# harryjfowen/PointsToWood

Measured on AMD Instinct MI355X. Metric: classified points/sec, higher is better.
Workload: dtype f16x3

## Files before the change

pointstowood_amd/csrc/p2w_hgemm.h:

```cpp
#pragma once
#include "p2w_common.h"
#include <type_traits>

typedef float f32x16 __attribute__((ext_vector_type(16)));
typedef _Float16 h8 __attribute__((ext_vector_type(8)));
typedef __bf16 bf8 __attribute__((ext_vector_type(8)));
typedef __fp16 hpair __attribute__((ext_vector_type(2)));
typedef _Float16 hpairn __attribute__((ext_vector_type(2)));
typedef __bf16 bpair __attribute__((ext_vector_type(2)));
typedef float fpair __attribute__((ext_vector_type(2)));
typedef __attribute__((address_space(3))) void* lds_vp;
typedef const __attribute__((address_space(1))) void* glb_vp;

constexpr int H_BK = 32;
constexpr int SA_EPI_COLS = 1024;

template <int PREC> struct HCfg {
    static constexpr int planes = PREC == 0 ? 2 : 1;
    static constexpr int kslab = PREC == 0 ? 32 : 64;
    static constexpr int kalign = PREC == 0 ? 32 : 64;
};

template <int PREC>
__device__ __forceinline__ f32x16 h_mfma(h8 a, h8 b, f32x16 c) {
// ... 56 lines not shown
        w.y = pack_pair<PREC>(v[2], v[3]);
        *reinterpret_cast<uint2*>(base + row * (size_t)ldh + col) = w;
    }
}

__device__ __forceinline__ bool tile_coords_at(int L, int nMt, int nNt, int* mt, int* nt, int mode = 0) {
    const int xcd = L & 7, w = L >> 3;
    if (mode == 0) {
        *mt = xcd + 8 * (w / nNt);
        *nt = w % nNt;
        return *mt < nMt;
    }
    if (nNt >= 8) {
        const int cpx = (nNt + 7) >> 3;
        *mt = w / cpx;
        *nt = xcd + 8 * (w % cpx);
        return *mt < nMt && *nt < nNt;
    }
    const int r = 8 / nNt;
    *nt = xcd % nNt;
    *mt = xcd / nNt + r * w;
    return *mt < nMt;
}
__device__ __forceinline__ bool tile_coords(int nMt, int nNt, int* mt, int* nt, int mode = 0) {
    return tile_coords_at(blockIdx.x, nMt, nNt, mt, nt, mode);
}
static inline int tile_grid(int nMt, int nNt, int mode = 0) {
    if (mode == 0) return 8 * ((nMt + 7) / 8) * nNt;
    if (nNt >= 8) return 8 * nMt * ((nNt + 7) / 8);
    const int r = 8 / nNt;
    return 8 * ((nMt + r - 1) / r);
}
static inline int p2w_cu_count() {
    int dev = 0, n = 256;
    if (hipGetDevice(&dev) == hipSuccess) hipDeviceGetAttribute(&n, hipDeviceAttributeMultiprocessorCount, dev);
    return n > 0 ? n : 256;
}

constexpr int RI_DEPTH = 2;
struct EpiArgs {
    const float *bias, *sc0, *sh0, *sc1, *sh1, *residual;
    int ldr, relu0, relu1, relu2, relu_final;
    const _Float16* res_h;
    unsigned* range;
    const int4* imeta;
};
__device__ __forceinline__ void range_commit(unsigned* __restrict__ dst, bool over, bool seen, int lane) {
    if (lane == 0) {
        unsigned* p = dst + (blockIdx.x & (P2W_RANGE_SLOTS - 1)) * 64;
        if (over) p[0] = 1u;
        if (seen) p[1] = 1u;
    }
}
__device__ __forceinline__ float nan_max(float a, float b) { return __builtin_elementwise_maximum(a, b); }
__device__ __forceinline__ void range_commit_max(unsigned* __restrict__ dst, float m, int lane) {
    range_commit(dst, __ballot(!(m <= P2W_RANGE_HI)) != 0ull, __ballot(m > P2W_RANGE_LO) != 0ull, lane);
}
template <int PREC>
__device__ __forceinline__ fpair h_load2(const _Float16* __restrict__ base, unsigned ldh, unsigned row, unsigned col) {
    if constexpr (PREC == 0) {
        const _Float16* p = base + (size_t)row * (2 * ldh) + 64 * (col >> 5) + (col & 31);
        const hpairn hi = *reinterpret_cast<const hpairn*>(p), lo = *reinterpret_cast<const hpairn*>(p + 32);
        return fpair{(float)hi[0] + (float)lo[0], (float)hi[1] + (float)lo[1]};
    } else if constexpr (PREC == 1) {
        const hpairn v = *reinterpret_cast<const hpairn*>(base + (size_t)row * ldh + col);
        return fpair{(float)v[0], (float)v[1]};
    } else {
        const bpair v = *reinterpret_cast<const bpair*>(base + (size_t)row * ldh + col);
        return fpair{(float)v[0], (float)v[1]};
    }
}
struct OutArgs { float* f32; int ldo; _Float16* h2; int ldh; int hcols; const float* dotw; float* part; int ldpart; };

__device__ __forceinline__ float row16_sum(float v) {
    asm volatile("s_nop 4\n\t"
                 "v_add_f32_dpp %0, %0, %0 quad_perm:[1,0,3,2] row_mask:0xf bank_mask:0xf bound_ctrl:1\n\ts_nop 1\n\t"
                 "v_add_f32_dpp %0, %0, %0 quad_perm:[2,3,0,1] row_mask:0xf bank_mask:0xf bound_ctrl:1\n\ts_nop 1\n\t"
                 "v_add_f32_dpp %0, %0, %0 row_half_mirror row_mask:0xf bank_mask:0xf bound_ctrl:1\n\ts_nop 1\n\t"
                 "v_add_f32_dpp %0, %0, %0 row_mirror row_mask:0xf bank_mask:0xf bound_ctrl:1\n\ts_nop 1"
                 : "+v"(v));
    return v;
}

__device__ __forceinline__ int w_stage_row16(int rho) {
    const int t = rho >> 4, c = rho & 15;
    return 32 * (t >> 1) + 2 * c + (t & 1);
}

template <int PREC, int RT16, int CT16, int EF, bool DOTK = false>
__device__ __forceinline__ void gemm_epilogue_16(const f32x4 (&acc)[RT16][CT16], const EpiArgs& ep, float wscale, int row0, int col0,
                                                 int lane, int M, int N, const OutArgs& o, bool seen_report = true) {
    static_assert(CT16 % 2 == 0, "column tiles come in interleaved pairs");
    constexpr bool GEN = EF < 0;
    constexpr int JQ = CT16 / 2, NSTEP = RT16 * 4;
    const bool R0 = GEN ? ep.relu0 != 0 : (EF & 1) != 0, S0 = GEN ? ep.sc0 != nullptr : (EF & 2) != 0;
    const bool R1 = GEN ? ep.relu1 != 0 : (EF & 4) != 0, S1 = GEN ? ep.sc1 != nullptr : (EF & 8) != 0;
    const bool R2 = GEN ? ep.relu2 != 0 : (EF & 16) != 0;
    const bool RES = !DOTK && (GEN ? (ep.residual != nullptr || ep.res_h != nullptr) : (EF & 32) != 0);
    const bool RF = GEN ? ep.relu_final != 0 : (EF & 64) != 0, OF = GEN ? o.f32 != nullptr : (EF & 128) != 0;
    const bool OH = GEN ? o.h2 != nullptr : (EF & 256) != 0;
    const bool RH = RES && (GEN ? ep.res_h != nullptr : (EF & 1024) != 0);
    constexpr bool RI_OK = !DOTK && RT16 <= 4;
    const bool RI = RI_OK && RES && (GEN ? ep.imeta != nullptr : (EF & 2048) != 0);
    const bool DOT = DOTK && (GEN ? o.dotw != nullptr : (EF & 512) != 0);
    const int c16 = lane & 15, kg = lane >> 4;
    const int cb = col0 + 2 * c16;
    fpair bias[JQ], s0[JQ], t0[JQ], s1[JQ], t1[JQ], dw[JQ];
#pragma unroll
    for (int jq = 0; jq < JQ; ++jq) {
        const int c = cb + 32 * jq;
        bias[jq] = fpair{0.f, 0.f}; s0[jq] = fpair{1.f, 1.f}; t0[jq] = fpair{0.f, 0.f}; s1[jq] = fpair{1.f, 1.f}; t1[jq] = fpair{0.f, 0.f};
        dw[jq] = fpair{0.f, 0.f};
        if constexpr (GEN) {
#pragma unroll
            for (int e = 0; e < 2; ++e)
                if (c + e < N) {
                    if (ep.bias) bias[jq][e] = ep.bias[c + e];
                    if (S0) { s0[jq][e] = ep.sc0[c + e]; t0[jq][e] = ep.sh0[c + e]; }
                    if (S1) { s1[jq][e] = ep.sc1[c + e]; t1[jq][e] = ep.sh1[c + e]; }
                    if (DOT) dw[jq][e] = o.dotw[c + e];
                }
        } else {
            if (DOT) dw[jq] = *reinterpret_cast<const fpair*>(o.dotw + c);
            if (ep.bias) bias[jq] = *reinterpret_cast<const fpair*>(ep.bias + c);
            if (S0) { s0[jq] = *reinterpret_cast<const fpair*>(ep.sc0 + c); t0[jq] = *reinterpret_cast<const fpair*>(ep.sh0 + c); }
            if (S1) { s1[jq] = *reinterpret_cast<const fpair*>(ep.sc1 + c); t1[jq] = *reinterpret_cast<const fpair*>(ep.sh1 + c); }
        }
    }
    auto row_of = [&](int st) { return row0 + 16 * (st >> 2) + 4 * kg + (st & 3); };
    auto value = [&](float a, float b, float s0v, float t0v, float s1v, float t1v, float res) {
        float v = fmaf(a, wscale, b);
        if (R0) v = fmaxf(v, 0.f);
        if (S0) v = fmaf(v, s0v, t0v);
        if (R1) v = fmaxf(v, 0.f);
        if (S1) v = fmaf(v, s1v, t1v);
        if (R2) v = fmaxf(v, 0.f);
        if (RES) v += res;
        if (RF) v = fmaxf(v, 0.f);
        return v;
    };
    fpair rcur[JQ], rnxt[JQ];
    constexpr int RI_D = RI_OK ? (RI_DEPTH < NSTEP ? RI_DEPTH : NSTEP) : 1;
    fpair z0r[RI_D][RI_OK ? JQ : 1], z1r[RI_D][RI_OK ? JQ : 1];
    float a0r[RI_D], a1r[RI_D];
    int4 m_nxt = make_int4(0, 0, 0, 0);
    auto load_zrows = [&](int slot, const int4& mt) {
        const float* p0 = ep.residual + ((unsigned)mt.x * (unsigned)ep.ldr + (unsigned)cb);
        const float* p1 = ep.residual + ((unsigned)mt.y * (unsigned)ep.ldr + (unsigned)cb);
#pragma unroll
        for (int jq = 0; jq < (RI_OK ? JQ : 1); ++jq) {
            z0r[slot][jq] = *reinterpret_cast<const fpair*>(p0 + 32 * jq);
            z1r[slot][jq] = *reinterpret_cast<const fpair*>(p1 + 32 * jq);
        }
        a0r[slot] = __int_as_float(mt.z); a1r[slot] = __int_as_float(mt.w);
    };
    auto load_res = [&](fpair (&dst)[JQ], int st) {
        if (RH) {
#pragma unroll
            for (int jq = 0; jq < JQ; ++jq) dst[jq] = h_load2<PREC>(ep.res_h, (unsigned)ep.ldr, (unsigned)row_of(st), (unsigned)(cb + 32 * jq));
        } else {
            const float* rp = ep.residual + ((unsigned)row_of(st) * (unsigned)ep.ldr + (unsigned)cb);
#pragma unroll
            for (int jq = 0; jq < JQ; ++jq) dst[jq] = *reinterpret_cast<const fpair*>(rp + 32 * jq);
        }
    };
#pragma unroll
    for (int jq = 0; jq < JQ; ++jq) { rcur[jq] = fpair{0.f, 0.f}; rnxt[jq] = fpair{0.f, 0.f}; }
    if constexpr (!GEN) {
        if constexpr (RI_OK) {
            if (RI) {
                int4 m0[RI_D];
#pragma unroll
                for (int d = 0; d < RI_D; ++d) m0[d] = ep.imeta[row_of(d)];
                if (RI_D < NSTEP) m_nxt = ep.imeta[row_of(RI_D)];
#pragma unroll
                for (int d = 0; d < RI_D; ++d) load_zrows(d, m0[d]);
            }
        }
        if (RES && !RI) load_res(rcur, 0);
    }
    float dot4[4] = {0.f, 0.f, 0.f, 0.f};
    unsigned long long r_over = 0ull, r_seen = 0ull;
    float m4 = 0.f;
#pragma unroll
    for (int st = 0; st < NSTEP; ++st) {
        const int it = st >> 2, reg = st & 3;
        const int row = row_of(st);
        if constexpr (!GEN) {
            if constexpr (RI_OK) {
                if (RI) {
#pragma unroll
                    for (int jq = 0; jq < JQ; ++jq)
                        rcur[jq] = fpair{fmaf(a1r[st % RI_D], z1r[st % RI_D][jq][0], a0r[st % RI_D] * z0r[st % RI_D][jq][0]),
                                         fmaf(a1r[st % RI_D], z1r[st % RI_D][jq][1], a0r[st % RI_D] * z0r[st % RI_D][jq][1])};
                    if (st + RI_D < NSTEP) {
                        load_zrows(st % RI_D, m_nxt);
                        if (st + RI_D + 1 < NSTEP) m_nxt = ep.imeta[row_of(st + RI_D + 1)];
                    }
                }
            }
            if (RES && !RI && st + 1 < NSTEP) load_res(rnxt, st + 1);
            __builtin_amdgcn_sched_barrier(0);
            float* fp = OF ? o.f32 + ((unsigned)row * (unsigned)o.ldo + (unsigned)cb) : nullptr;
            _Float16* hp = nullptr;
            if (OH) {
                if constexpr (PREC == 0) hp = o.h2 + ((unsigned)row * (unsigned)(2 * o.ldh) + (unsigned)(64 * (cb >> 5) + (cb & 31)));
                else hp = o.h2 + ((unsigned)row * (unsigned)o.ldh + (unsigned)cb);
            }
            float dsum = 0.f;
#pragma unroll
            for (int jq = 0; jq < JQ; ++jq) {
                const float va = value(acc[it][2 * jq][reg], bias[jq][0], s0[jq][0], t0[jq][0], s1[jq][0], t1[jq][0], rcur[jq][0]);
                const float vb = value(acc[it][2 * jq + 1][reg], bias[jq][1], s0[jq][1], t0[jq][1], s1[jq][1], t1[jq][1], rcur[jq][1]);
                m4 = nan_max(nan_max(m4, fabsf(va)), fabsf(vb));
                if (DOT) dsum = fmaf(vb, dw[jq][1], fmaf(va, dw[jq][0], dsum));
                if (OF) *reinterpret_cast<fpair*>(fp + 32 * jq) = fpair{va, vb};
                if (OH) {
                    if constexpr (PREC == 0) {
                        unsigned hw, lw;
                        split_pair(va, vb, hw, lw);
                        *reinterpret_cast<unsigned*>(hp + 64 * jq) = hw;
                        *reinterpret_cast<unsigned*>(hp + 64 * jq + 32) = lw;
                    } else {
                        *reinterpret_cast<unsigned*>(hp + 32 * jq) = pack_pair<PREC>(va, vb);
                    }
                }
            }
            if (reg == 3) {
                r_over |= __ballot(!(m4 <= P2W_RANGE_HI));
                r_seen |= __ballot(m4 > P2W_RANGE_LO);
                m4 = 0.f;
            }
            if (DOT) {
                dot4[reg] = row16_sum(dsum);
                if (reg == 3 && c16 == 0)
                    *reinterpret_cast<float4*>(o.part + ((unsigned)(col0 >> 6) * (unsigned)o.ldpart + (unsigned)(row - 3))) =
                        make_float4(dot4[0], dot4[1], dot4[2], dot4[3]);
            }
            if (RES && !RI) {
#pragma unroll
                for (int jq = 0; jq < JQ; ++jq) rcur[jq] = rnxt[jq];
            }
        } else {
            float dsum = 0.f;
            if (row < M) {
                int4 mt = make_int4(0, 0, 0, 0);
                if constexpr (RI_OK) {
                    if (RI) mt = ep.imeta[row];
                }
#pragma unroll
                for (int jq = 0; jq < JQ; ++jq) {
                    const int c = cb + 32 * jq;
                    float v[2];
#pragma unroll
                    for (int e = 0; e < 2; ++e) {
                        const bool cv = c + e < N;
                        float res = 0.f;
                        if (RI && cv) res = fmaf(__int_as_float(mt.w), ep.residual[(size_t)mt.y * ep.ldr + c + e], __int_as_float(mt.z) * ep.residual[(size_t)mt.x * ep.ldr + c + e]);
                        else if (RES && cv) res = RH ? h_load2<PREC>(ep.res_h, (unsigned)ep.ldr, (unsigned)row, (unsigned)c)[e] : ep.residual[(size_t)row * ep.ldr + c + e];
                        v[e] = value(acc[it][2 * jq + e][reg], bias[jq][e], s0[jq][e], t0[jq][e], s1[jq][e], t1[jq][e], res);
                        if (!cv) v[e] = 0.f;
                        if (OF && cv) o.f32[(size_t)row * o.ldo + c + e] = v[e];
                    }
                    {
                        const float m2 = nan_max(fabsf(v[0]), fabsf(v[1]));
                        r_over |= __ballot(!(m2 <= P2W_RANGE_HI));
                        r_seen |= __ballot(m2 > P2W_RANGE_LO);
                    }
                    if (DOT) dsum = fmaf(v[1], dw[jq][1], fmaf(v[0], dw[jq][0], dsum));
                    if (OH && c < o.hcols) h_store2<PREC>(o.h2, o.ldh, row, c, v[0], v[1]);
                }
            }
            if (DOT) {
                dsum = row16_sum(dsum);
                if (row < M && c16 == 0 && col0 < N) o.part[(size_t)(col0 >> 6) * o.ldpart + row] = dsum;
            }
        }
    }
    if (ep.range) range_commit(ep.range, r_over != 0ull, seen_report && r_seen != 0ull, lane);
}

constexpr int p2w_vmcnt_imm(int n) { return (n & 15) | (7 << 4) | (15 << 8) | ((n >> 4) << 14); }

template <int PREC, int RT16, int CT16, bool WAIT_OLDER = false, bool DOTK = false>
__device__ __forceinline__ void gemm_epilogue_dispatch16(const f32x4 (&acc)[RT16][CT16], const EpiArgs& ep, float wscale, int row0,
                                                         int col0, int lane, int M, int N, const OutArgs& o, int ef,
                                                         bool seen_report = true) {
    const bool full = (row0 + 16 * RT16 <= M) && (col0 + 16 * CT16 <= N) && ef != 0;
    if (full) {
        if constexpr (DOTK) {
            if (ef == 513) {
                gemm_epilogue_16<PREC, RT16, CT16, 513, true>(acc, ep, wscale, row0, col0, lane, M, N, o, seen_report);
                if constexpr (WAIT_OLDER) __builtin_amdgcn_s_waitcnt(p2w_vmcnt_imm(RT16 < 63 ? RT16 : 63));
                return;
            }
        } else
        switch (ef) {
#define P2W_EPI_CASE(E) case E: { \
            gemm_epilogue_16<PREC, RT16, CT16, E>(acc, ep, wscale, row0, col0, lane, M, N, o, seen_report); \
            constexpr int n_st = RT16 * 4 * (CT16 / 2) * (((E) & 128 ? 1 : 0) + ((E) & 256 ? (PREC == 0 ? 2 : 1) : 0)) ; \
            if constexpr (WAIT_OLDER) __builtin_amdgcn_s_waitcnt(p2w_vmcnt_imm(n_st < 63 ? n_st : 63)); \
            return; }
            P2W_EPI_CASE(128) P2W_EPI_CASE(257) P2W_EPI_CASE(263) P2W_EPI_CASE(287) P2W_EPI_CASE(224)
            P2W_EPI_CASE(131) P2W_EPI_CASE(259) P2W_EPI_CASE(387) P2W_EPI_CASE(129)
            P2W_EPI_CASE(480) P2W_EPI_CASE(1376) P2W_EPI_CASE(1504)
#undef P2W_EPI_CASE
            case 2400:
                if constexpr (!DOTK && RT16 <= 4) {
                    gemm_epilogue_16<PREC, RT16, CT16, 2400>(acc, ep, wscale, row0, col0, lane, M, N, o, seen_report);
                    constexpr int n_st = RT16 * 4 * (CT16 / 2) * (PREC == 0 ? 2 : 1);
                    if constexpr (WAIT_OLDER) __builtin_amdgcn_s_waitcnt(p2w_vmcnt_imm(n_st < 63 ? n_st : 63));
                    return;
                }
                break;
            default: break;
        }
    }
    gemm_epilogue_16<PREC, RT16, CT16, -1, DOTK>(acc, ep, wscale, row0, col0, lane, M, N, o, seen_report);
    if constexpr (WAIT_OLDER) __builtin_amdgcn_s_waitcnt(p2w_vmcnt_imm(0));
}

template <int PREC, int WR, int WC, int RT, int CT, bool DOTK, bool SK>
__device__ __forceinline__ void gemm_hp_body(const _Float16* __restrict__ A, int ldh_a, const _Float16* __restrict__ Wh, float wscale,
                                             int M, int N, int Kpad, int nMt, int nNt, int nvb, const EpiArgs& ep, const OutArgs& o,
                                             int ef, int tmode, int sk_S, float* __restrict__ skws) {
    constexpr int KS = HCfg<PREC>::kslab;
    constexpr int BM = 32 * RT * WR, BN = 32 * CT * WC, NW = WR * WC;
    constexpr int A_CH = 8 * BM, STAGE_CH = A_CH + 8 * BN;
    constexpr bool HALF = NW == 8;
    constexpr int NWI = HALF ? NW / 2 : NW;
    constexpr int NI = STAGE_CH / 64 / NWI;
    static_assert(STAGE_CH % (64 * NWI) == 0, "stage must split evenly over the issuing waves");
    __shared__ __attribute__((aligned(16))) char S[2 * STAGE_CH * 16];
    const int tid = threadIdx.x, lane = tid & 63;
    const int wave = __builtin_amdgcn_readfirstlane(tid >> 6), wr = wave / WC, wc = wave % WC;
    const size_t a_pitch = (size_t)HCfg<PREC>::planes * ldh_a, w_pitch = (size_t)HCfg<PREC>::planes * Kpad;
    auto next_tile = [&](int& L, int& mt_, int& nt_) {
        while (L < nvb) {
            if (tile_coords_at(L, nMt, nNt, &mt_, &nt_, tmode)) return true;
            L += gridDim.x;
        }
        return false;
    };
    const int nslab = Kpad / KS;
    int L = blockIdx.x, mt, nt;
    int sk_s0 = 0, sk_s1 = 0, sk_piece = 0;
    if constexpr (SK) {
        const int P = nvb * sk_S, per_xcd = (P + 7) >> 3;
        const int w = blockIdx.x >> 3;
        sk_piece = (blockIdx.x & 7) * per_xcd + w;
        if (w >= per_xcd || sk_piece >= P) return;
        const int j = sk_piece / nvb, r = sk_piece - j * nvb;
        sk_s0 = (int)((long long)j * nslab / sk_S);
        sk_s1 = (int)((long long)(j + 1) * nslab / sk_S);
        if (sk_s0 >= sk_s1) return;
        mt = r / nNt; nt = r - mt * nNt;
    } else if (!next_tile(L, mt, nt)) {
        return;
    }

    const _Float16* src[NI];
    auto setup_src = [&](int mt_, int nt_) {
#pragma unroll
        for (int i = 0; i < NI; ++i) {
            const int g = (wave % NWI) + NWI * i;
            const int row = 8 * g + (lane >> 3);
            const int c = (lane & 7) ^ ((row >> 1) & 7);
            if (g < BM / 8) src[i] = A + (size_t)min(mt_ * BM + row, M - 1) * a_pitch + 8 * c;
            else src[i] = Wh + (size_t)(nt_ * BN + w_stage_row16(row - BM)) * w_pitch + 8 * c;
        }
    };
    const unsigned lds_base = (unsigned)(uintptr_t)(lds_vp)S;
    auto issue_piece = [&](int i, int stage, int k0) {
        const int g = (wave % NWI) + NWI * i;
        const unsigned dst = lds_base + (unsigned)(stage * STAGE_CH + g * 64) * 16u;
        asm volatile("s_mov_b32 m0, %1\n\ts_nop 0\n\tglobal_load_lds_dwordx4 %0, off"
                     :: "v"(src[i] + k0), "s"(dst) : "m0", "memory");
    };
    const bool issuer = wave < NWI;
    constexpr int RT16 = 2 * RT, CT16 = 2 * CT;
    const int r16 = lane & 15, kg = lane >> 4;
    int offA[RT16], offB[CT16];
#pragma unroll
    for (int t = 0; t < RT16; ++t) {
        const int ra = wr * 32 * RT + 16 * t + r16;
        offA[t] = (ra * 8 + (kg ^ ((ra >> 1) & 7))) * 16;
    }
#pragma unroll
    for (int t = 0; t < CT16; ++t) {
        const int rb = BM + wc * 32 * CT + 16 * t + r16;
        offB[t] = (rb * 8 + (kg ^ ((rb >> 1) & 7))) * 16;
    }
    setup_src(mt, nt);
    if (issuer) {
#pragma unroll
        for (int i = 0; i < NI; ++i) issue_piece(i, 0, SK ? sk_s0 * 64 : 0);
    }
    int gs = 0;
    bool landed = false;
    f32x4 acc[RT16][CT16];
    h8 ah[RT16 / 2], al[RT16 / 2], bh[CT16], bl[CT16];
    auto slab = [&](int s, auto last_c, int mtn, int ntn) {
        constexpr bool LAST = decltype(last_c)::value;
        asm volatile("" ::: "memory");
        if (landed) __builtin_amdgcn_s_waitcnt(0xC07F);
        else __builtin_amdgcn_s_waitcnt(0x0070);
        landed = false;
        __builtin_amdgcn_s_barrier();
        asm volatile("" ::: "memory");
        if constexpr (LAST) setup_src(mtn, ntn);
        constexpr int HR = RT16 / 2;
        constexpr int NG = 2 * HR * CT16;
        constexpr int GAP = (NG / (2 * NI)) > 0 ? NG / (2 * NI) : 1;
        const int k_next = LAST ? 0 : (s + 1) * 64;
        if constexpr (HALF) {
            if (issuer) {
#pragma unroll
                for (int i = 0; i < NI; ++i) issue_piece(i, (gs + 1) & 1, k_next);
            }
        }
        const char* st = S + (size_t)(gs & 1) * STAGE_CH * 16;
#pragma unroll
        for (int t = 0; t < CT16; ++t) {
            bh[t] = *reinterpret_cast<const h8*>(st + offB[t]);
            bl[t] = *reinterpret_cast<const h8*>(st + (offB[t] ^ 64));
        }
#pragma unroll
        for (int hh = 0; hh < 2; ++hh) {
#pragma unroll
            for (int t = 0; t < HR; ++t) {
                ah[t] = *reinterpret_cast<const h8*>(st + offA[hh * HR + t]);
                al[t] = *reinterpret_cast<const h8*>(st + (offA[hh * HR + t] ^ 64));
            }
#pragma unroll
            for (int i = 0; i < HR; ++i)
#pragma unroll
                for (int j = 0; j < CT16; ++j) {
                    f32x4& c = acc[hh * HR + i][j];
                    if constexpr (PREC == 0) {
                        c = h_mfma16<PREC>(al[i], bh[j], c);
                        c = h_mfma16<PREC>(ah[i], bl[j], c);
                        c = h_mfma16<PREC>(ah[i], bh[j], c);
                    } else {
                        c = h_mfma16<PREC>(ah[i], bh[j], c);
                        c = h_mfma16<PREC>(al[i], bl[j], c);
                    }
                    if constexpr (!HALF) {
                        const int g = (hh * HR + i) * CT16 + j;
                        if ((g % GAP) == GAP - 1 && g / GAP < NI) {
                            issue_piece(g / GAP, (gs + 1) & 1, k_next);
                            __builtin_amdgcn_sched_barrier(0);
                        }
                    }
                }
        }
        ++gs;
    };
    if constexpr (SK) {
#pragma unroll
        for (int i = 0; i < RT16; ++i)
#pragma unroll
            for (int j = 0; j < CT16; ++j) acc[i][j] = f32x4{0.f, 0.f, 0.f, 0.f};
        for (int s = sk_s0; s + 1 < sk_s1; ++s) slab(s, std::false_type{}, 0, 0);
        slab(sk_s1 - 1, std::true_type{}, mt, nt);
        f32x4* dst = reinterpret_cast<f32x4*>(skws) + (size_t)sk_piece * (size_t)(BM * BN / 4) + tid;
#pragma unroll
        for (int i = 0; i < RT16; ++i)
#pragma unroll
            for (int j = 0; j < CT16; ++j) dst[(i * CT16 + j) * (64 * NW)] = acc[i][j];
    } else {
    while (true) {
        int Ln = L + gridDim.x, mtn = mt, ntn = nt;
        const bool more = next_tile(Ln, mtn, ntn);
        if (!more) { mtn = mt; ntn = nt; }
#pragma unroll
        for (int i = 0; i < RT16; ++i)
#pragma unroll
            for (int j = 0; j < CT16; ++j) acc[i][j] = f32x4{0.f, 0.f, 0.f, 0.f};
        for (int s = 0; s + 1 < nslab; ++s) slab(s, std::false_type{}, 0, 0);
        slab(nslab - 1, std::true_type{}, mtn, ntn);
        gemm_epilogue_dispatch16<PREC, RT16, CT16, true, DOTK>(acc, ep, wscale, mt * BM + wr * 32 * RT, nt * BN + wc * 32 * CT, lane, M, N, o, ef,
                                                               gs == nslab && wave == 0);
        landed = true;
        if (!more) break;
        L = Ln; mt = mtn; nt = ntn;
    }
    }
    asm volatile("s_waitcnt vmcnt(0)" ::: "memory");
}

template <int PREC, int WR, int WC, int RT, int CT, bool DOTK = false>
__global__ __launch_bounds__(64 * WR * WC, 2) void gemm_hp_kernel(const _Float16* __restrict__ A, int ldh_a,
                                                               const _Float16* __restrict__ Wh, float wscale, int M, int N,
                                                               int Kpad, int nMt, int nNt, int nvb, EpiArgs ep, OutArgs o, int ef,
                                                               int tmode) {
    gemm_hp_body<PREC, WR, WC, RT, CT, DOTK, false>(A, ldh_a, Wh, wscale, M, N, Kpad, nMt, nNt, nvb, ep, o, ef, tmode, 0, nullptr);
}

template <int PREC>
__global__ __launch_bounds__(256, 3) void gemm_hp64_kernel(const _Float16* __restrict__ A, int ldh_a, const _Float16* __restrict__ Wh,
                                                        float wscale, int M, int N, int Kpad, int nMt, int nNt, int nvb, EpiArgs ep,
                                                        OutArgs o, int ef, int tmode) {
    gemm_hp_body<PREC, 2, 2, 1, 2, false, false>(A, ldh_a, Wh, wscale, M, N, Kpad, nMt, nNt, nvb, ep, o, ef, tmode, 0, nullptr);
}

template <int PREC, int WR, int WC, int RT, int CT>
__global__ __launch_bounds__(64 * WR * WC, 2) void gemm_hp_sk_kernel(const _Float16* __restrict__ A, int ldh_a,
                                                                  const _Float16* __restrict__ Wh, int M, int Kpad, int nNt,
                                                                  int tiles, int S, float* __restrict__ skws) {
    const EpiArgs ep = {};
    const OutArgs o = {};
    gemm_hp_body<PREC, WR, WC, RT, CT, false, true>(A, ldh_a, Wh, 1.f, M, 0, Kpad, 0, nNt, tiles, ep, o, 0, 0, S, skws);
}

template <int PREC, int WR, int WC, int RT, int CT>
__global__ __launch_bounds__(64 * WR * WC) void gemm_hp_skfix_kernel(const float* __restrict__ skws, int tiles, int S, int nslab, int nNt,
                                                                      float wscale, int M, int N, EpiArgs ep, OutArgs o, int ef) {
    constexpr int BM = 32 * RT * WR, BN = 32 * CT * WC, NW = WR * WC, RT16 = 2 * RT, CT16 = 2 * CT;
    const int tid = threadIdx.x, lane = tid & 63;
    const int wave = __builtin_amdgcn_readfirstlane(tid >> 6), wr = wave / WC, wc = wave % WC;
    const int r = blockIdx.x / RT16, i = blockIdx.x - r * RT16;
    f32x4 acc[1][CT16];
#pragma unroll
    for (int j = 0; j < CT16; ++j) acc[0][j] = f32x4{0.f, 0.f, 0.f, 0.f};
    for (int p = 0; p < S; ++p) {
        if ((int)((long long)p * nslab / S) >= (int)((long long)(p + 1) * nslab / S)) continue;
        const f32x4* src = reinterpret_cast<const f32x4*>(skws) + (size_t)(p * tiles + r) * (size_t)(BM * BN / 4) + tid;
#pragma unroll
        for (int jj = 0; jj < CT16; ++jj) acc[0][jj] += src[(i * CT16 + jj) * (64 * NW)];
    }
    const int mt = r / nNt, nt = r - mt * nNt;
    gemm_epilogue_dispatch16<PREC, 1, CT16, false, false>(acc, ep, wscale, mt * BM + wr * 32 * RT + 16 * i, nt * BN + wc * 32 * CT, lane, M, N, o, ef);
}

template <int PREC>
static int32_t launch_gemm_h(const _Float16* Ah, int32_t ldh_a, const _Float16* Wp, float wscale, int32_t M, int32_t N, int32_t K,
                             const EpiArgs& ep, float* out_f32, int32_t ldo, _Float16* out_h2, int32_t ldh_o, int32_t flags,
                             hipStream_t stream, const float* dotw = nullptr, float* part = nullptr, int32_t ldpart = 0,
                             float* skws = nullptr, size_t skws_bytes = 0, int sk_S = 0) {
    constexpr int KA = HCfg<PREC>::kalign;
    const int Npad = (N + 255) / 256 * 256, Kpad = (K + KA - 1) / KA * KA;
    if (ep.imeta) flags = (flags & ~P2W_GEMM_TILE_256) | P2W_GEMM_TILE_128;
    if ((ldh_a % KA) != 0 || ldh_a < Kpad) return P2W_EINVAL;
    if (out_h2 && (ldh_o & 7)) return P2W_EINVAL;
    const int hcols = ldh_o < (N + KA - 1) / KA * KA ? ldh_o : (N + KA - 1) / KA * KA;
    OutArgs o = {out_f32, ldo, out_h2, ldh_o, hcols, dotw, part, ldpart};
    const int n_cu = p2w_cu_count();
    auto pick_big = [&](int rows) {
        const long tiles256 = (long)p2w_cdiv(rows, 256) * (Npad / 256);
        const long rounds = (tiles256 + n_cu - 1) / n_cu;
        const bool fills = tiles256 * 100 >= rounds * n_cu * 78;
        bool b = N >= 256 && (N % 256) == 0 && tiles256 * 4 >= 3 * n_cu && fills;
        if (flags & P2W_GEMM_TILE_256) b = true;
        if (flags & P2W_GEMM_TILE_128) b = false;
        return b;
    };
    const bool big = pick_big(M);
    bool t64 = false;
    if (!dotw && sk_S == 0 && !ep.imeta && !(flags & (P2W_GEMM_TILE_128 | P2W_GEMM_TILE_256 | P2W_GEMM_NO_TILE_64))) {
        if (flags & P2W_GEMM_TILE_64) t64 = true;
        else if (K <= 1024 && N <= 192) t64 = true;
        else if (K <= 1024 && !big) {
            const long nNt1 = p2w_cdiv(N, 128), T128 = (long)p2w_cdiv(M, 128) * nNt1, T64 = (long)p2w_cdiv(M, 64) * nNt1;
            const long S128 = 2L * n_cu, S64 = 3L * n_cu;
            const double w128 = (double)((T128 + S128 - 1) / S128 * S128) / (double)T128, w64 = (double)((T64 + S64 - 1) / S64 * S64) / (double)T64;
            t64 = T128 <= 2 * S128 && w128 >= 1.3 * w64;
        }
    }
    if (sk_S == 0 && skws && !dotw && !t64 && !(flags & P2W_GEMM_NO_STREAMK)) {
        const int nslab = Kpad / HCfg<PREC>::kslab;
        const double f = PREC == 0 ? 1.0 : 0.7, ts1 = 0.9 * f, ts2 = 1.65 * f, tsb = 2.25 * f;
        auto t_small = [&](long tiles) { return tiles > n_cu ? ts2 : ts1; };
        auto t_big = [&](long tiles) { return tiles >= n_cu ? tsb : (0.75 * f + (tsb - 0.75 * f) * (double)tiles / n_cu); };
        auto one_launch = [&](bool b, int rows) {
            const long T = b ? (long)p2w_cdiv(rows, 256) * (Npad / 256) : (long)p2w_cdiv(rows, 128) * p2w_cdiv(N, 128);
            const long G = b ? n_cu : 2 * n_cu, qq = T / G, R = T % G;
            return (double)nslab * ((double)qq * (b ? tsb : ts2) + (R ? (b ? t_big(R) : t_small(R)) : 0.0));
        };
        const bool big_ok = N >= 256 && (N % 256) == 0;
        double best_cost = one_launch(big, M);
        int best_mode = 0, best_rows_full = 0, best_S = 0;
        bool best_big = big, sk_big = big, tail_big = false;
        double sk_cost = 1e30;
        int sk_rows_full = 0, sk_S_best = 0;
        const size_t piece_b = (size_t)128 * 128 * 4;
        for (int cand = 0; cand < 2; ++cand) {
            const bool b = cand == 0;
            if (b && !(N >= 256 && (N % 256) == 0)) continue;
            if ((flags & P2W_GEMM_TILE_256) && !b) continue;
            if ((flags & P2W_GEMM_TILE_128) && b) continue;
            const int BMm = b ? 256 : 128, G_m = n_cu * (b ? 1 : 2);
            const int nNt_m = b ? Npad / 256 : p2w_cdiv(N, 128), nMt_m = p2w_cdiv(M, BMm);
            const long T = (long)nMt_m * nNt_m, q = T / G_m;
            const int mt_full = (int)((q * G_m) / nNt_m);
            if ((long)mt_full * nNt_m >= T) continue;
            if (q == 0 && b != big) continue;
            const int rows_full = mt_full * BMm, m_t = M - rows_full;
            const double main_t = (double)q * nslab * (b ? tsb : ts2) + (q > 0 ? 4.0 : 0.0);
            const long T_t = (long)p2w_cdiv(m_t, 128) * p2w_cdiv(N, 128);
            if (q > 0) {
                for (int tb = 0; tb < 2; ++tb) {
                    if (tb == 1 && (!big_ok || (flags & P2W_GEMM_TILE_128))) continue;
                    if (tb == 0 && (flags & P2W_GEMM_TILE_256)) continue;
                    const double c = main_t + one_launch(tb == 1, m_t);
                    if (c < 0.95 * best_cost) { best_cost = c; best_mode = 1; best_rows_full = rows_full; best_big = b; best_S = 0; tail_big = tb == 1; }
                }
            }
            for (int S = 2; S <= nslab && T_t * S <= 2 * n_cu; ++S) {
                if ((size_t)(T_t * S) * piece_b > skws_bytes) break;
                const double c = main_t + (double)((nslab + S - 1) / S) * 1.0 * f + 18.0 + (double)(T_t * S) * piece_b * 2.0 / 8.0e6;
                if (c < sk_cost) { sk_cost = c; sk_rows_full = rows_full; sk_big = b; sk_S_best = S; }
            }
        }
        if (sk_S_best > 0 && (sk_cost < 0.9 * best_cost || (flags & P2W_GEMM_STREAMK))) {
            best_mode = 2; best_rows_full = sk_rows_full; best_big = sk_big; best_S = sk_S_best;
        }
        if (best_mode != 0) {
            constexpr int PL = HCfg<PREC>::planes;
            const int fl = (flags & ~(P2W_GEMM_STREAMK | P2W_GEMM_TILE_128 | P2W_GEMM_TILE_256)) | P2W_GEMM_NO_STREAMK;
            const int rows_full = best_rows_full, m_t = M - rows_full;
            if (rows_full > 0) {
                const int32_t rc = launch_gemm_h<PREC>(Ah, ldh_a, Wp, wscale, rows_full, N, K, ep, out_f32, ldo, out_h2, ldh_o,
                                                       fl | (best_big ? P2W_GEMM_TILE_256 : P2W_GEMM_TILE_128), stream);
                if (rc != P2W_OK) return rc;
            }
            const size_t r0 = (size_t)rows_full;
            EpiArgs ept = ep;
            if (ept.imeta) ept.imeta += r0;
            else if (ept.residual) ept.residual += r0 * ep.ldr;
            if (ept.res_h) ept.res_h += r0 * PL * ep.ldr;
            return launch_gemm_h<PREC>(Ah + r0 * PL * ldh_a, ldh_a, Wp, wscale, m_t, N, K, ept, out_f32 ? out_f32 + r0 * ldo : nullptr, ldo,
                                       out_h2 ? out_h2 + r0 * PL * ldh_o : nullptr, ldh_o,
                                       best_mode == 2 ? fl : (fl | (tail_big ? P2W_GEMM_TILE_256 : P2W_GEMM_TILE_128)), stream, nullptr, nullptr, 0,
                                       best_mode == 2 ? skws : nullptr, skws_bytes, best_mode == 2 ? best_S : 0);
        }
    }
    int ef = (ep.relu0 ? 1 : 0) | (ep.sc0 ? 2 : 0) | (ep.relu1 ? 4 : 0) | (ep.sc1 ? 8 : 0) | (ep.relu2 ? 16 : 0) |
             ((ep.residual || ep.res_h) ? 32 : 0) | (ep.relu_final ? 64 : 0) | (out_f32 ? 128 : 0) | (out_h2 ? 256 : 0) | (dotw ? 512 : 0) |
             (ep.res_h ? 1024 : 0) | (ep.imeta ? 2048 : 0);
    const size_t lim = (size_t)1 << 31;
    if ((size_t)M * (size_t)(ldo > 2 * ldh_o ? ldo : 2 * ldh_o) >= lim || ((ep.residual || ep.res_h) && !ep.imeta && (size_t)M * (size_t)ep.ldr * (ep.res_h ? 2 : 1) >= lim) ||
        (N & 1) || (flags & P2W_GEMM_GENERIC_EPI))
        ef = 0;
    auto odd8 = [](const void* q) { return (reinterpret_cast<uintptr_t>(q) & 7) != 0; };
    if ((out_f32 && ((ldo & 1) || odd8(out_f32))) || (ep.residual && ((ep.ldr & 1) || odd8(ep.residual))) || odd8(ep.bias) ||
        (ep.res_h && ((ep.ldr & 7) || (reinterpret_cast<uintptr_t>(ep.res_h) & 15))) ||
        odd8(ep.sc0) || odd8(ep.sh0) || odd8(ep.sc1) || odd8(ep.sh1) || odd8(dotw) || (part && ((ldpart & 3) || (reinterpret_cast<uintptr_t>(part) & 15))))
        ef = 0;
    const size_t w_bytes = (size_t)N * Kpad * 2 * HCfg<PREC>::planes, a_bytes = (size_t)M * Kpad * 2 * HCfg<PREC>::planes;
    auto pick_mode = [&](int nNtx, int nMtx, int per_cu) {
        const bool ok = nNtx >= 8 || (nNtx > 0 && 8 % nNtx == 0);
        if (!ok) return 0;
        if (flags & P2W_GEMM_ORDER_ROWS) return 0;
        if (flags & P2W_GEMM_ORDER_COLS) return 1;
        const size_t l2_keep = (size_t)3 * 1024 * 1024;
        const int wpx = n_cu / 8 * per_cu;
        const int R = wpx / nNtx > 0 ? wpx / nNtx : 1;
        const int rows_px = p2w_cdiv(nMtx, 8), xcds = nMtx < 8 ? nMtx : 8;
        const size_t t_rows = a_bytes * (size_t)p2w_cdiv(nNtx, wpx) + w_bytes * xcds * (w_bytes <= l2_keep ? 1 : p2w_cdiv(rows_px, R));
        size_t t_cols;
        if (nNtx >= 8) {
            const int cpx = p2w_cdiv(nNtx, 8), Rc = wpx / cpx > 0 ? wpx / cpx : 1;
            t_cols = a_bytes * 8 + w_bytes * (w_bytes / 8 <= l2_keep ? 1 : p2w_cdiv(nMtx, Rc));
        } else {
            t_cols = a_bytes * nNtx + w_bytes * 8 / nNtx;
        }
        return t_cols * 10 < t_rows * 9 ? 1 : 0;
    };
    auto pgrid = [&](int nvb, int per_cu) {
        const int cap = n_cu * per_cu;
        int g = nvb < cap ? nvb : cap;
        if (g >= 8) g &= ~7;
        return g;
    };
    if (sk_S > 0) {
        const int nslab = Kpad / HCfg<PREC>::kslab, nNt1 = p2w_cdiv(N, 128), T_t = p2w_cdiv(M, 128) * nNt1;
        gemm_hp_sk_kernel<PREC, 2, 2, 2, 2><<<8 * p2w_cdiv(T_t * sk_S, 8), 256, 0, stream>>>(Ah, ldh_a, Wp, M, Kpad, nNt1, T_t, sk_S, skws);
        gemm_hp_skfix_kernel<PREC, 2, 2, 2, 2><<<T_t * 4, 256, 0, stream>>>(skws, T_t, sk_S, nslab, nNt1, wscale, M, N, ep, o, ef);
    } else if (t64) {
        const int nMt = p2w_cdiv(M, 64), nNt1 = p2w_cdiv(N, 128);
        const int tm = pick_mode(nNt1, nMt, 3), nvb = tile_grid(nMt, nNt1, tm);
        gemm_hp64_kernel<PREC><<<pgrid(nvb, 3), 256, 0, stream>>>(Ah, ldh_a, Wp, wscale, M, N, Kpad, nMt, nNt1, nvb, ep, o, ef, tm);
    } else if (big) {
        const int nMt = p2w_cdiv(M, 256), nNt2 = Npad / 256;
        const int tm = pick_mode(nNt2, nMt, 1), nvb = tile_grid(nMt, nNt2, tm);
        if (dotw) gemm_hp_kernel<PREC, 2, 4, 4, 2, true><<<pgrid(nvb, 1), 512, 0, stream>>>(Ah, ldh_a, Wp, wscale, M, N, Kpad, nMt, nNt2, nvb, ep, o, ef, tm);
        else gemm_hp_kernel<PREC, 2, 4, 4, 2><<<pgrid(nvb, 1), 512, 0, stream>>>(Ah, ldh_a, Wp, wscale, M, N, Kpad, nMt, nNt2, nvb, ep, o, ef, tm);
    } else {
        const int nMt = p2w_cdiv(M, 128), nNt1 = p2w_cdiv(N, 128);
        const int tm = pick_mode(nNt1, nMt, 2), nvb = tile_grid(nMt, nNt1, tm);
        if (dotw) gemm_hp_kernel<PREC, 2, 2, 2, 2, true><<<pgrid(nvb, 2), 256, 0, stream>>>(Ah, ldh_a, Wp, wscale, M, N, Kpad, nMt, nNt1, nvb, ep, o, ef, tm);
        else gemm_hp_kernel<PREC, 2, 2, 2, 2><<<pgrid(nvb, 2), 256, 0, stream>>>(Ah, ldh_a, Wp, wscale, M, N, Kpad, nMt, nNt1, nvb, ep, o, ef, tm);
    }
    return P2W_LAUNCH_STATUS();
}

template <int RT, int GPT> struct SaEpiRegs { float bias[2], s[2], t[2]; int dsc[RT][GPT]; };
template <int PREC, int RT, int G>
__device__ __forceinline__ void sa_epilogue_regs(const f32x16 (&acc)[RT][2], float wscale, int n0, int wc, int lane,
                                                 const SaEpiRegs<RT, 32 / G>& e, int C2, float* __restrict__ out, int ldo,
                                                 _Float16* __restrict__ out_h2, int ldh, float& amax) {
    static_assert(G == 32 || G == 8, "one or four targets per 32-row tile");
    constexpr int GPT = 32 / G;
    const int h = lane >> 5;
#pragma unroll
    for (int i = 0; i < RT; ++i) {
#pragma unroll
        for (int q = 0; q < GPT; ++q) {
            const int dsc = __builtin_amdgcn_readfirstlane(e.dsc[i][q]);
            if (dsc < 0) continue;
            const int tgt = dsc >> 6, d = dsc & 63;
#pragma unroll
            for (int j = 0; j < 2; ++j) {
                const int col = n0 + wc * 64 + j * 32 + (lane & 31);
                const bool cv = col < C2;
                const float sgn = e.s[j] < 0.f ? -1.f : 1.f;
                const fpair sg2 = {sgn, sgn};
                float ext;
                if constexpr (G == 32) {
                    if (d >= 32) {
                        fpair p[8];
#pragma unroll
                        for (int u = 0; u < 8; ++u) p[u] = fpair{acc[i][j][2 * u], acc[i][j][2 * u + 1]} * sg2;
                        float m0 = fmaxf(fmaxf(p[0][0], p[0][1]), p[1][0]);
                        float m1 = fmaxf(fmaxf(p[1][1], p[2][0]), p[2][1]);
                        float m2 = fmaxf(fmaxf(p[3][0], p[3][1]), p[4][0]);
                        float m3 = fmaxf(fmaxf(p[4][1], p[5][0]), p[5][1]);
                        m0 = fmaxf(fmaxf(m0, p[6][0]), p[6][1]);
                        m1 = fmaxf(fmaxf(m1, p[7][0]), p[7][1]);
                        ext = fmaxf(fmaxf(m0, m1), fmaxf(m2, m3));
// ... 407 lines not shown
```

Measured before the change: 20.00 million.

## Widen GEMM epilogue to four adjacent columns per lane with 16-byte stores

Changes the weight staging permutation so each lane's four column tiles map to four adjacent output columns, letting the epilogue load bias/scale/residual as float4 and write f32/f16 outputs with 16- or 8-byte vector stores instead of pairs. This cuts the number of memory instructions in the epilogue and the vmcnt wait depth. The specialised path now requires N divisible by 4 and 16-byte alignment, so more shapes fall back to the generic epilogue; it also re-runs source setup each tile for RT16==8.

```diff
diff --git a/pointstowood_amd/csrc/p2w_hgemm.h b/pointstowood_amd/csrc/p2w_hgemm.h
--- a/pointstowood_amd/csrc/p2w_hgemm.h
+++ b/pointstowood_amd/csrc/p2w_hgemm.h
@@ -162,17 +162,39 @@
     return v;
 }
 
+constexpr int EPI_CT16 = 4;
 __device__ __forceinline__ int w_stage_row16(int rho) {
     const int t = rho >> 4, c = rho & 15;
-    return 32 * (t >> 1) + 2 * c + (t & 1);
+    return 64 * (t >> 2) + 4 * c + (t & 3);
+}
+template <int PREC>
+__device__ __forceinline__ f32x4 h_load4(const _Float16* __restrict__ base, unsigned ldh, unsigned row, unsigned col) {
+    typedef _Float16 h4 __attribute__((ext_vector_type(4)));
+    typedef __bf16 b4 __attribute__((ext_vector_type(4)));
+    if constexpr (PREC == 0) {
+        const _Float16* p = base + (size_t)row * (2 * ldh) + 64 * (col >> 5) + (col & 31);
+        const h4 hi = *reinterpret_cast<const h4*>(p), lo = *reinterpret_cast<const h4*>(p + 32);
+        return f32x4{(float)hi[0] + (float)lo[0], (float)hi[1] + (float)lo[1], (float)hi[2] + (float)lo[2], (float)hi[3] + (float)lo[3]};
+    } else if constexpr (PREC == 1) {
+        const h4 v = *reinterpret_cast<const h4*>(base + (size_t)row * ldh + col);
+        return f32x4{(float)v[0], (float)v[1], (float)v[2], (float)v[3]};
+    } else {
+        const b4 v = *reinterpret_cast<const b4*>(base + (size_t)row * ldh + col);
+        return f32x4{(float)v[0], (float)v[1], (float)v[2], (float)v[3]};
+    }
+}
+
+template <int PREC, int RT16>
+constexpr int gemm_epilogue_stores(int ef) {
+    return RT16 * 4 * ((ef & 128 ? 1 : 0) + (ef & 256 ? HCfg<PREC>::planes : 0)) + (ef & 512 ? RT16 : 0);
 }
 
 template <int PREC, int RT16, int CT16, int EF, bool DOTK = false>
 __device__ __forceinline__ void gemm_epilogue_16(const f32x4 (&acc)[RT16][CT16], const EpiArgs& ep, float wscale, int row0, int col0,
                                                  int lane, int M, int N, const OutArgs& o, bool seen_report = true) {
-    static_assert(CT16 % 2 == 0, "column tiles come in interleaved pairs");
+    static_assert(CT16 == EPI_CT16, "a lane owns the four adjacent columns of its wave's four column tiles");
     constexpr bool GEN = EF < 0;
-    constexpr int JQ = CT16 / 2, NSTEP = RT16 * 4;
+    constexpr int NSTEP = RT16 * 4;
     const bool R0 = GEN ? ep.relu0 != 0 : (EF & 1) != 0, S0 = GEN ? ep.sc0 != nullptr : (EF & 2) != 0;
     const bool R1 = GEN ? ep.relu1 != 0 : (EF & 4) != 0, S1 = GEN ? ep.sc1 != nullptr : (EF & 8) != 0;
     const bool R2 = GEN ? ep.relu2 != 0 : (EF & 16) != 0;
@@ -184,28 +206,30 @@
     const bool RI = RI_OK && RES && (GEN ? ep.imeta != nullptr : (EF & 2048) != 0);
     const bool DOT = DOTK && (GEN ? o.dotw != nullptr : (EF & 512) != 0);
     const int c16 = lane & 15, kg = lane >> 4;
-    const int cb = col0 + 2 * c16;
-    fpair bias[JQ], s0[JQ], t0[JQ], s1[JQ], t1[JQ], dw[JQ];
-#pragma unroll
-    for (int jq = 0; jq < JQ; ++jq) {
-        const int c = cb + 32 * jq;
-        bias[jq] = fpair{0.f, 0.f}; s0[jq] = fpair{1.f, 1.f}; t0[jq] = fpair{0.f, 0.f}; s1[jq] = fpair{1.f, 1.f}; t1[jq] = fpair{0.f, 0.f};
-        dw[jq] = fpair{0.f, 0.f};
-        if constexpr (GEN) {
-#pragma unroll
-            for (int e = 0; e < 2; ++e)
-                if (c + e < N) {
-                    if (ep.bias) bias[jq][e] = ep.bias[c + e];
-                    if (S0) { s0[jq][e] = ep.sc0[c + e]; t0[jq][e] = ep.sh0[c + e]; }
-                    if (S1) { s1[jq][e] = ep.sc1[c + e]; t1[jq][e] = ep.sh1[c + e]; }
-                    if (DOT) dw[jq][e] = o.dotw[c + e];
-                }
-        } else {
-            if (DOT) dw[jq] = *reinterpret_cast<const fpair*>(o.dotw + c);
-            if (ep.bias) bias[jq] = *reinterpret_cast<const fpair*>(ep.bias + c);
-            if (S0) { s0[jq] = *reinterpret_cast<const fpair*>(ep.sc0 + c); t0[jq] = *reinterpret_cast<const fpair*>(ep.sh0 + c); }
-            if (S1) { s1[jq] = *reinterpret_cast<const fpair*>(ep.sc1 + c); t1[jq] = *reinterpret_cast<const fpair*>(ep.sh1 + c); }
-        }
+    const int cb = col0 + 4 * c16;
+    const f32x4 zero4 = {0.f, 0.f, 0.f, 0.f};
+    float bias[4], s0[4], t0[4], s1[4], t1[4], dw[4];
+#pragma unroll
+    for (int e = 0; e < 4; ++e) { bias[e] = 0.f; s0[e] = 1.f; t0[e] = 0.f; s1[e] = 1.f; t1[e] = 0.f; dw[e] = 0.f; }
+    if constexpr (GEN) {
+#pragma unroll
+        for (int e = 0; e < 4; ++e)
+            if (cb + e < N) {
+                if (ep.bias) bias[e] = ep.bias[cb + e];
+                if (S0) { s0[e] = ep.sc0[cb + e]; t0[e] = ep.sh0[cb + e]; }
+                if (S1) { s1[e] = ep.sc1[cb + e]; t1[e] = ep.sh1[cb + e]; }
+                if (DOT) dw[e] = o.dotw[cb + e];
+            }
+    } else {
+        auto load4 = [&](float (&dst)[4], const float* src) {
+            const f32x4 q = *reinterpret_cast<const f32x4*>(src + cb);
+#pragma unroll
+            for (int e = 0; e < 4; ++e) dst[e] = q[e];
+        };
+        if (DOT) load4(dw, o.dotw);
+        if (ep.bias) load4(bias, ep.bias);
+        if (S0) { load4(s0, ep.sc0); load4(t0, ep.sh0); }
+        if (S1) { load4(s1, ep.sc1); load4(t1, ep.sh1); }
     }
     auto row_of = [&](int st) { return row0 + 16 * (st >> 2) + 4 * kg + (st & 3); };
     auto value = [&](float a, float b, float s0v, float t0v, float s1v, float t1v, float res) {
@@ -219,33 +243,20 @@
         if (RF) v = fmaxf(v, 0.f);
         return v;
     };
-    fpair rcur[JQ], rnxt[JQ];
+    f32x4 rcur = zero4, rnxt = zero4;
     constexpr int RI_D = RI_OK ? (RI_DEPTH < NSTEP ? RI_DEPTH : NSTEP) : 1;
-    fpair z0r[RI_D][RI_OK ? JQ : 1], z1r[RI_D][RI_OK ? JQ : 1];
+    f32x4 z0r[RI_D], z1r[RI_D];
     float a0r[RI_D], a1r[RI_D];
     int4 m_nxt = make_int4(0, 0, 0, 0);
     auto load_zrows = [&](int slot, const int4& mt) {
-        const float* p0 = ep.residual + ((unsigned)mt.x * (unsigned)ep.ldr + (unsigned)cb);
-        const float* p1 = ep.residual + ((unsigned)mt.y * (unsigned)ep.ldr + (unsigned)cb);
-#pragma unroll
-        for (int jq = 0; jq < (RI_OK ? JQ : 1); ++jq) {
-            z0r[slot][jq] = *reinterpret_cast<const fpair*>(p0 + 32 * jq);
-            z1r[slot][jq] = *reinterpret_cast<const fpair*>(p1 + 32 * jq);
-        }
+        z0r[slot] = *reinterpret_cast<const f32x4*>(ep.residual + ((unsigned)mt.x * (unsigned)ep.ldr + (unsigned)cb));
+        z1r[slot] = *reinterpret_cast<const f32x4*>(ep.residual + ((unsigned)mt.y * (unsigned)ep.ldr + (unsigned)cb));
         a0r[slot] = __int_as_float(mt.z); a1r[slot] = __int_as_float(mt.w);
     };
-    auto load_res = [&](fpair (&dst)[JQ], int st) {
-        if (RH) {
-#pragma unroll
-            for (int jq = 0; jq < JQ; ++jq) dst[jq] = h_load2<PREC>(ep.res_h, (unsigned)ep.ldr, (unsigned)row_of(st), (unsigned)(cb + 32 * jq));
-        } else {
-            const float* rp = ep.residual + ((unsigned)row_of(st) * (unsigned)ep.ldr + (unsigned)cb);
-#pragma unroll
-            for (int jq = 0; jq < JQ; ++jq) dst[jq] = *reinterpret_cast<const fpair*>(rp + 32 * jq);
-        }
-    };
-#pragma unroll
-    for (int jq = 0; jq < JQ; ++jq) { rcur[jq] = fpair{0.f, 0.f}; rnxt[jq] = fpair{0.f, 0.f}; }
+    auto load_res = [&](f32x4& dst, int st) {
+        if (RH) dst = h_load4<PREC>(ep.res_h, (unsigned)ep.ldr, (unsigned)row_of(st), (unsigned)cb);
+        else dst = *reinterpret_cast<const f32x4*>(ep.residual + ((unsigned)row_of(st) * (unsigned)ep.ldr + (unsigned)cb));
+    };
     if constexpr (!GEN) {
         if constexpr (RI_OK) {
             if (RI) {
@@ -270,9 +281,7 @@
             if constexpr (RI_OK) {
                 if (RI) {
 #pragma unroll
-                    for (int jq = 0; jq < JQ; ++jq)
-                        rcur[jq] = fpair{fmaf(a1r[st % RI_D], z1r[st % RI_D][jq][0], a0r[st % RI_D] * z0r[st % RI_D][jq][0]),
-                                         fmaf(a1r[st % RI_D], z1r[st % RI_D][jq][1], a0r[st % RI_D] * z0r[st % RI_D][jq][1])};
+                    for (int e = 0; e < 4; ++e) rcur[e] = fmaf(a1r[st % RI_D], z1r[st % RI_D][e], a0r[st % RI_D] * z0r[st % RI_D][e]);
                     if (st + RI_D < NSTEP) {
                         load_zrows(st % RI_D, m_nxt);
                         if (st + RI_D + 1 < NSTEP) m_nxt = ep.imeta[row_of(st + RI_D + 1)];
@@ -281,29 +290,26 @@
             }
             if (RES && !RI && st + 1 < NSTEP) load_res(rnxt, st + 1);
             __builtin_amdgcn_sched_barrier(0);
-            float* fp = OF ? o.f32 + ((unsigned)row * (unsigned)o.ldo + (unsigned)cb) : nullptr;
-            _Float16* hp = nullptr;
+            float v[4], dsum = 0.f;
+#pragma unroll
+            for (int e = 0; e < 4; e += 2) {
+                v[e] = value(acc[it][e][reg], bias[e], s0[e], t0[e], s1[e], t1[e], rcur[e]);
+                v[e + 1] = value(acc[it][e + 1][reg], bias[e + 1], s0[e + 1], t0[e + 1], s1[e + 1], t1[e + 1], rcur[e + 1]);
+                m4 = nan_max(nan_max(m4, fabsf(v[e])), fabsf(v[e + 1]));
+                if (DOT) dsum = fmaf(v[e + 1], dw[e + 1], fmaf(v[e], dw[e], dsum));
+            }
+            if (OF) *reinterpret_cast<f32x4*>(o.f32 + ((unsigned)row * (unsigned)o.ldo + (unsigned)cb)) = f32x4{v[0], v[1], v[2], v[3]};
             if (OH) {
-                if constexpr (PREC == 0) hp = o.h2 + ((unsigned)row * (unsigned)(2 * o.ldh) + (unsigned)(64 * (cb >> 5) + (cb & 31)));
-                else hp = o.h2 + ((unsigned)row * (unsigned)o.ldh + (unsigned)cb);
-            }
-            float dsum = 0.f;
-#pragma unroll
-            for (int jq = 0; jq < JQ; ++jq) {
-                const float va = value(acc[it][2 * jq][reg], bias[jq][0], s0[jq][0], t0[jq][0], s1[jq][0], t1[jq][0], rcur[jq][0]);
-                const float vb = value(acc[it][2 * jq + 1][reg], bias[jq][1], s0[jq][1], t0[jq][1], s1[jq][1], t1[jq][1], rcur[jq][1]);
-                m4 = nan_max(nan_max(m4, fabsf(va)), fabsf(vb));
-                if (DOT) dsum = fmaf(vb, dw[jq][1], fmaf(va, dw[jq][0], dsum));
-                if (OF) *reinterpret_cast<fpair*>(fp + 32 * jq) = fpair{va, vb};
-                if (OH) {
-                    if constexpr (PREC == 0) {
-                        unsigned hw, lw;
-                        split_pair(va, vb, hw, lw);
-                        *reinterpret_cast<unsigned*>(hp + 64 * jq) = hw;
-                        *reinterpret_cast<unsigned*>(hp + 64 * jq + 32) = lw;
-                    } else {
-                        *reinterpret_cast<unsigned*>(hp + 32 * jq) = pack_pair<PREC>(va, vb);
-                    }
+                if constexpr (PREC == 0) {
+                    _Float16* hp = o.h2 + ((unsigned)row * (unsigned)(2 * o.ldh) + (unsigned)(64 * (cb >> 5) + (cb & 31)));
+                    uint2 hw, lw;
+                    split_pair(v[0], v[1], hw.x, lw.x);
+                    split_pair(v[2], v[3], hw.y, lw.y);
+                    *reinterpret_cast<uint2*>(hp) = hw;
+                    *reinterpret_cast<uint2*>(hp + 32) = lw;
+                } else {
+                    *reinterpret_cast<uint2*>(o.h2 + ((unsigned)row * (unsigned)o.ldh + (unsigned)cb)) =
+                        make_uint2(pack_pair<PREC>(v[0], v[1]), pack_pair<PREC>(v[2], v[3]));
                 }
             }
             if (reg == 3) {
@@ -317,10 +323,7 @@
                     *reinterpret_cast<float4*>(o.part + ((unsigned)(col0 >> 6) * (unsigned)o.ldpart + (unsigned)(row - 3))) =
                         make_float4(dot4[0], dot4[1], dot4[2], dot4[3]);
             }
-            if (RES && !RI) {
-#pragma unroll
-                for (int jq = 0; jq < JQ; ++jq) rcur[jq] = rnxt[jq];
-            }
+            if (RES && !RI) rcur = rnxt;
         } else {
             float dsum = 0.f;
             if (row < M) {
@@ -328,27 +331,28 @@
                 if constexpr (RI_OK) {
                     if (RI) mt = ep.imeta[row];
                 }
-#pragma unroll
-                for (int jq = 0; jq < JQ; ++jq) {
-                    const int c = cb + 32 * jq;
-                    float v[2];
-#pragma unroll
-                    for (int e = 0; e < 2; ++e) {
-                        const bool cv = c + e < N;
-                        float res = 0.f;
-                        if (RI && cv) res = fmaf(__int_as_float(mt.w), ep.residual[(size_t)mt.y * ep.ldr + c + e], __int_as_float(mt.z) * ep.residual[(size_t)mt.x * ep.ldr + c + e]);
-                        else if (RES && cv) res = RH ? h_load2<PREC>(ep.res_h, (unsigned)ep.ldr, (unsigned)row, (unsigned)c)[e] : ep.residual[(size_t)row * ep.ldr + c + e];
-                        v[e] = value(acc[it][2 * jq + e][reg], bias[jq][e], s0[jq][e], t0[jq][e], s1[jq][e], t1[jq][e], res);
-                        if (!cv) v[e] = 0.f;
-                        if (OF && cv) o.f32[(size_t)row * o.ldo + c + e] = v[e];
-                    }
-                    {
-                        const float m2 = nan_max(fabsf(v[0]), fabsf(v[1]));
-                        r_over |= __ballot(!(m2 <= P2W_RANGE_HI));
-                        r_seen |= __ballot(m2 > P2W_RANGE_LO);
-                    }
-                    if (DOT) dsum = fmaf(v[1], dw[jq][1], fmaf(v[0], dw[jq][0], dsum));
-                    if (OH && c < o.hcols) h_store2<PREC>(o.h2, o.ldh, row, c, v[0], v[1]);
+                float v[4];
+#pragma unroll
+                for (int e = 0; e < 4; ++e) {
+                    const int c = cb + e;
+                    const bool cv = c < N;
+                    float res = 0.f;
+                    if (RI && cv) res = fmaf(__int_as_float(mt.w), ep.residual[(size_t)mt.y * ep.ldr + c], __int_as_float(mt.z) * ep.residual[(size_t)mt.x * ep.ldr + c]);
+                    else if (RES && cv) res = RH ? h_load2<PREC>(ep.res_h, (unsigned)ep.ldr, (unsigned)row, (unsigned)(c & ~1))[e & 1] : ep.residual[(size_t)row * ep.ldr + c];
+                    v[e] = value(acc[it][e][reg], bias[e], s0[e], t0[e], s1[e], t1[e], res);
+                    if (!cv) v[e] = 0.f;
+                    if (OF && cv) o.f32[(size_t)row * o.ldo + c] = v[e];
+                }
+                {
+                    const float m2 = nan_max(nan_max(fabsf(v[0]), fabsf(v[1])), nan_max(fabsf(v[2]), fabsf(v[3])));
+                    r_over |= __ballot(!(m2 <= P2W_RANGE_HI));
+                    r_seen |= __ballot(m2 > P2W_RANGE_LO);
+                }
+                if (DOT) dsum = fmaf(v[3], dw[3], fmaf(v[2], dw[2], fmaf(v[1], dw[1], v[0] * dw[0])));
+                if (OH) {
+#pragma unroll
+                    for (int e = 0; e < 4; e += 2)
+                        if (cb + e < o.hcols) h_store2<PREC>(o.h2, o.ldh, row, cb + e, v[e], v[e + 1]);
                 }
             }
             if (DOT) {
@@ -368,31 +372,22 @@
                                                          bool seen_report = true) {
     const bool full = (row0 + 16 * RT16 <= M) && (col0 + 16 * CT16 <= N) && ef != 0;
     if (full) {
-        if constexpr (DOTK) {
-            if (ef == 513) {
-                gemm_epilogue_16<PREC, RT16, CT16, 513, true>(acc, ep, wscale, row0, col0, lane, M, N, o, seen_report);
-                if constexpr (WAIT_OLDER) __builtin_amdgcn_s_waitcnt(p2w_vmcnt_imm(RT16 < 63 ? RT16 : 63));
-                return;
-            }
-        } else
         switch (ef) {
-#define P2W_EPI_CASE(E) case E: { \
-            gemm_epilogue_16<PREC, RT16, CT16, E>(acc, ep, wscale, row0, col0, lane, M, N, o, seen_report); \
-            constexpr int n_st = RT16 * 4 * (CT16 / 2) * (((E) & 128 ? 1 : 0) + ((E) & 256 ? (PREC == 0 ? 2 : 1) : 0)) ; \
-            if constexpr (WAIT_OLDER) __builtin_amdgcn_s_waitcnt(p2w_vmcnt_imm(n_st < 63 ? n_st : 63)); \
-            return; }
-            P2W_EPI_CASE(128) P2W_EPI_CASE(257) P2W_EPI_CASE(263) P2W_EPI_CASE(287) P2W_EPI_CASE(224)
-            P2W_EPI_CASE(131) P2W_EPI_CASE(259) P2W_EPI_CASE(387) P2W_EPI_CASE(129)
-            P2W_EPI_CASE(480) P2W_EPI_CASE(1376) P2W_EPI_CASE(1504)
+#define P2W_EPI_CASE(E, DK) case E: \
+            if constexpr (DOTK == (DK) && ((E) != 2400 || RT16 <= 4)) { \
+                gemm_epilogue_16<PREC, RT16, CT16, E, DK>(acc, ep, wscale, row0, col0, lane, M, N, o, seen_report); \
+                constexpr int n_st = gemm_epilogue_stores<PREC, RT16>(E); \
+                static_assert(n_st > 0, "every class stores something"); \
+                if constexpr (WAIT_OLDER) __builtin_amdgcn_s_waitcnt(p2w_vmcnt_imm(n_st < 63 ? n_st : 63)); \
+                return; \
+            } \
+            break;
+            P2W_EPI_CASE(513, true)
+            P2W_EPI_CASE(128, false) P2W_EPI_CASE(257, false) P2W_EPI_CASE(263, false) P2W_EPI_CASE(287, false) P2W_EPI_CASE(224, false)
+            P2W_EPI_CASE(131, false) P2W_EPI_CASE(259, false) P2W_EPI_CASE(387, false) P2W_EPI_CASE(129, false)
+            P2W_EPI_CASE(480, false) P2W_EPI_CASE(1376, false) P2W_EPI_CASE(1504, false)
+            P2W_EPI_CASE(2400, false)
 #undef P2W_EPI_CASE
-            case 2400:
-                if constexpr (!DOTK && RT16 <= 4) {
-                    gemm_epilogue_16<PREC, RT16, CT16, 2400>(acc, ep, wscale, row0, col0, lane, M, N, o, seen_report);
-                    constexpr int n_st = RT16 * 4 * (CT16 / 2) * (PREC == 0 ? 2 : 1);
-                    if constexpr (WAIT_OLDER) __builtin_amdgcn_s_waitcnt(p2w_vmcnt_imm(n_st < 63 ? n_st : 63));
-                    return;
-                }
-                break;
             default: break;
         }
     }
@@ -459,6 +454,7 @@
     };
     const bool issuer = wave < NWI;
     constexpr int RT16 = 2 * RT, CT16 = 2 * CT;
+    static_assert(CT16 == EPI_CT16, "w_stage_row16 deals a wave's 64 columns to four column tiles");
     const int r16 = lane & 15, kg = lane >> 4;
     int offA[RT16], offB[CT16];
 #pragma unroll
@@ -564,6 +560,10 @@
         landed = true;
         if (!more) break;
         L = Ln; mt = mtn; nt = ntn;
+        if constexpr (RT16 == 8) {
+            asm volatile("" : "+s"(mt), "+s"(nt));
+            setup_src(mt, nt);
+        }
     }
     }
     asm volatile("s_waitcnt vmcnt(0)" ::: "memory");
@@ -720,12 +720,12 @@
              (ep.res_h ? 1024 : 0) | (ep.imeta ? 2048 : 0);
     const size_t lim = (size_t)1 << 31;
     if ((size_t)M * (size_t)(ldo > 2 * ldh_o ? ldo : 2 * ldh_o) >= lim || ((ep.residual || ep.res_h) && !ep.imeta && (size_t)M * (size_t)ep.ldr * (ep.res_h ? 2 : 1) >= lim) ||
-        (N & 1) || (flags & P2W_GEMM_GENERIC_EPI))
+        (N & 3) || (flags & P2W_GEMM_GENERIC_EPI))
         ef = 0;
-    auto odd8 = [](const void* q) { return (reinterpret_cast<uintptr_t>(q) & 7) != 0; };
-    if ((out_f32 && ((ldo & 1) || odd8(out_f32))) || (ep.residual && ((ep.ldr & 1) || odd8(ep.residual))) || odd8(ep.bias) ||
-        (ep.res_h && ((ep.ldr & 7) || (reinterpret_cast<uintptr_t>(ep.res_h) & 15))) ||
-        odd8(ep.sc0) || odd8(ep.sh0) || odd8(ep.sc1) || odd8(ep.sh1) || odd8(dotw) || (part && ((ldpart & 3) || (reinterpret_cast<uintptr_t>(part) & 15))))
+    auto odd16 = [](const void* q) { return (reinterpret_cast<uintptr_t>(q) & 15) != 0; };
+    if ((out_f32 && ((ldo & 3) || odd16(out_f32))) || (ep.residual && ((ep.ldr & 3) || odd16(ep.residual))) || odd16(ep.bias) ||
+        (out_h2 && (reinterpret_cast<uintptr_t>(out_h2) & 7)) || (ep.res_h && ((ep.ldr & 7) || odd16(ep.res_h))) ||
+        odd16(ep.sc0) || odd16(ep.sh0) || odd16(ep.sc1) || odd16(ep.sh1) || odd16(dotw) || (part && ((ldpart & 3) || odd16(part))))
         ef = 0;
     const size_t w_bytes = (size_t)N * Kpad * 2 * HCfg<PREC>::planes, a_bytes = (size_t)M * Kpad * 2 * HCfg<PREC>::planes;
     auto pick_mode = [&](int nNtx, int nMtx, int per_cu) {
```

After: 19.84 million. Within noise of the previous version (-0.8%).
